# Vahe1994/AQLM

Measured on AMD Instinct MI355X. Metric: QuantizedLinear 1x16g8 matvec algorithmic GB/s (bs=1, Llama-3-8B shapes 4096->4096/11008), higher is better.
Workload: dtype f16; 1 GPU; decode step = 32 blocks x {4096->4096, 4096->11008} 1x16g8 matvec, bs=1, 64 distinct layers (own codes + codebook), 564 MB algorithmic bytes/step, hipGraph replay; scheme=1x16g8, batch=1, kernels=prepacked slice-bucketed gemv (layers of >= 0.5 M codes: both shapes), parallelism=single GPU, packed_bytes=1190264832, canonical_code_bytes=494927872

## Files before the change

aqlm_amd/_native.py:

```python
from __future__ import annotations

import ctypes
import os

_HERE = os.path.dirname(os.path.abspath(__file__))
LIB_PATH = os.environ.get("AQLM_AMD_HIP_LIB") or os.path.join(_HERE, "libaqlm_hip.so")
ABI_VERSION = 9

F16, BF16 = 0, 1
F32 = 2
E_INVALID, E_UNSUPPORTED = -1, -2
MAX_GEMV_BATCH = 8
OP_GEMM_1X16_MFMA = 1
OP_GEMV_1X16_PACKED = 3
OP_GEMV_8X8_LUT = 4
OP_GEMM_KX8_MFMA = 6
OP_GEMV_1X16_G16_PACKED = 5

MAX_SEGMENTS = 4
MAX_ROUTED_PAIRS = 64
MAX_ROUTED_EXPERTS = 256
ROUTED_ENTRY_WORDS = 4
MAX_GROUPED_PAIRS = 1 << 18
GROUPED_TILE_PAIRS = (16, 32, 64, 128)
# ... 228 lines not shown

def check(rc: int, what: str = "") -> None:
    if rc == 0:
        return
    msg = last_error() or what
    if rc == E_UNSUPPORTED:
        raise NotImplementedError(msg)
    if rc == E_INVALID:
        raise ValueError(msg)
    raise AqlmHipError(f"HIP error {rc}: {msg}")


def set_tuning(key: str, value: int) -> None:
    check(lib.aqlm_hip_set_tuning(key.encode(), int(value)), "set_tuning")


def get_tuning(key: str) -> int:
    v = _ci(0)
    check(lib.aqlm_hip_get_tuning(key.encode(), ctypes.byref(v)), "get_tuning")
    return v.value


CAPTURE_OVERLAP_FIELDS = ("seen", "relaxed", "kept_conflict", "kept_window", "runs_broken", "api_failures",
                          "merged", "merge_refused", "nodes_added")


def capture_overlap_stats(reset: bool = False) -> dict:
    out = (ctypes.c_uint64 * len(CAPTURE_OVERLAP_FIELDS))()
    check(lib.aqlm_hip_capture_overlap_stats_ex(out, len(out)), "capture_overlap_stats")
    if reset:
        check(lib.aqlm_hip_capture_overlap_stats_ex(None, 0), "capture_overlap_stats")
    return dict(zip(CAPTURE_OVERLAP_FIELDS, (int(v) for v in out)))


def packed_image(desc: "PackedDesc", rows: int = 1, dtype: int = F16):
    lds, win = _sz(0), ctypes.c_uint32(0)
    check(lib.aqlm_hip_gemv_1x16_packed_image(ctypes.byref(desc), int(rows), int(dtype), 0, ctypes.byref(lds), ctypes.byref(win), None),
          "packed_image")
    return int(lds.value), int(win.value)


def packed_image_blocks_per_cu(desc: "PackedDesc", rows: int = 1, dtype: int = F16, probe_lds_bytes: int = 0) -> int:
    n = _ci(0)
    check(lib.aqlm_hip_gemv_1x16_packed_image(ctypes.byref(desc), int(rows), int(dtype), int(probe_lds_bytes), None, None, ctypes.byref(n)),
          "packed_image")
    return n.value
```

aqlm_amd/csrc/api.hip:

```cpp
#include <stdarg.h>
#include <string.h>

#include <algorithm>
#include <map>
#include <mutex>
#include <utility>

#include "aqlm_common.h"

namespace aqlm {

static thread_local char g_err[512] = "";

void set_last_error(const char* fmt, ...) {
  va_list ap;
  va_start(ap, fmt);
  vsnprintf(g_err, sizeof(g_err), fmt, ap);
  va_end(ap);
}

int check_hip(hipError_t e, const char* what) {
  if (e == hipSuccess) return 0;
  set_last_error("%s: %s (%d)", what, hipGetErrorString(e), (int)e);
  return (int)e;
// ... 33 lines not shown
  if (!strcmp(key, "kx8_xres_phased")) return &t.kx8_xres_phased;
  if (!strcmp(key, "kx8_phase_tpb")) return &t.kx8_phase_tpb;
  if (!strcmp(key, "kx8_phase_quads")) return &t.kx8_phase_quads;
  if (!strcmp(key, "kx8_multi_xres_min_rows")) return &t.kx8_multi_xres_min_rows;
  if (!strcmp(key, "kx8_ksplit")) return &t.kx8_ksplit;
  if (!strcmp(key, "kx8_rt")) return &t.kx8_rt;
  if (!strcmp(key, "scan_max_rows")) return &t.scan_max_rows;
  if (!strcmp(key, "scan_prefetch")) return &t.scan_prefetch;
  if (!strcmp(key, "gemm_debug")) return &t.gemm_debug;
  if (!strcmp(key, "gemm_store_nt")) return &t.gemm_store_nt;
  if (!strcmp(key, "force_generic")) return &t.force_generic;
  if (!strcmp(key, "packed_waves")) return &t.packed_waves;
  if (!strcmp(key, "packed_fused_finalize")) return &t.packed_fused_finalize;
  if (!strcmp(key, "packed_prefetch")) return &t.packed_prefetch;
  if (!strcmp(key, "packed_arrange")) return &t.packed_arrange;
  if (!strcmp(key, "packed_xcopies")) return &t.packed_xcopies;
  if (!strcmp(key, "packed_entry_bytes")) return &t.packed_entry_bytes;
  if (!strcmp(key, "packed_debug")) return &t.packed_debug;
  if (!strcmp(key, "packed_fill_rotate")) return &t.packed_fill_rotate;
  if (!strcmp(key, "packed_compact_window")) return &t.packed_compact_window;
  if (!strcmp(key, "packed_capture_window")) return &t.packed_capture_window;
  if (!strcmp(key, "packed_capture_min_run")) return &t.packed_capture_min_run;
  if (!strcmp(key, "packed_capture_merge")) return &t.packed_capture_merge;
  if (!strcmp(key, "packed_pipe")) return &t.packed_pipe;
  if (!strcmp(key, "packed_prefetch_waves")) return &t.packed_prefetch_waves;
  if (!strcmp(key, "packed_dequant_by_xcd")) return &t.packed_dequant_by_xcd;
  if (!strcmp(key, "lut_waves")) return &t.lut_waves;
  return nullptr;
}

namespace {
struct CaptureOverlapState {
  std::mutex mu;
  capture_overlap::Planner planner;
  uint64_t stats[9] = {0, 0, 0, 0, 0, 0, 0, 0, 0};
  bool off = false;
};
CaptureOverlapState& capture_state() {
  static CaptureOverlapState s;
  return s;
}
hipError_t set_capture_deps(hipStream_t stream, const std::vector<capture_overlap::NodeId>& nodes) {
  static_assert(sizeof(hipGraphNode_t) == sizeof(capture_overlap::NodeId), "a graph node handle is carried as a 64-bit id");
  std::vector<hipGraphNode_t> d;
  for (capture_overlap::NodeId n : nodes) d.push_back(reinterpret_cast<hipGraphNode_t>(static_cast<uintptr_t>(n)));
  return hipStreamUpdateCaptureDependencies(stream, d.empty() ? nullptr : d.data(), d.size(), hipStreamSetCaptureDependencies);
}
bool same_nodes(const std::vector<capture_overlap::NodeId>& a, const std::vector<capture_overlap::NodeId>& b) {
  return a.size() == b.size() && std::is_permutation(a.begin(), a.end(), b.begin());
}
bool read_capture(hipStream_t stream, bool& capturing, unsigned long long& id, std::vector<capture_overlap::NodeId>& deps, hipError_t& err) {
  hipStreamCaptureStatus st = hipStreamCaptureStatusNone;
  const hipGraphNode_t* d = nullptr;
  size_t n = 0;
  hipGraph_t graph = nullptr;
  err = hipStreamGetCaptureInfo_v2(stream, &st, &id, &graph, &d, &n);
  if (err != hipSuccess) return false;
  capturing = st == hipStreamCaptureStatusActive;
// ... 46 lines not shown
  }
  fail("hipStreamUpdateCaptureDependencies", e);
  s.planner.run(id_).reset();
  active_ = false;
}

int CaptureRelax::begin(uint64_t key, const void* member, size_t member_bytes) {
  if (!active_ || begun_) return 0;
  begun_ = true;
  const int merge = std::min(std::max(tuning().packed_capture_merge, 1), capture_overlap::kMaxMerge);
  if (merge > 1 && key != 0 && member) {
    key_ = key;
    member_.assign(static_cast<const unsigned char*>(member), static_cast<const unsigned char*>(member) + member_bytes);
  }
  CaptureOverlapState& s = capture_state();
  std::lock_guard<std::mutex> lock(s.mu);
  plan_ = s.planner.run(id_).plan(before_.data(), before_.size(), fp, tuning().packed_capture_window, tuning().packed_capture_min_run,
                                  key_, merge);
  if (plan_.merge) return plan_.member;
  apply_plan();
  return 0;
}

bool CaptureRelax::join(const hipKernelNodeParams* node) {
  if (!active_ || !begun_ || done_ || !plan_.merge) return false;
  CaptureOverlapState& s = capture_state();
  std::lock_guard<std::mutex> lock(s.mu);
  capture_overlap::Run& run = s.planner.run(id_);
  const hipError_t e = node && run.latest(plan_)
                           ? hipGraphKernelNodeSetParams(reinterpret_cast<hipGraphNode_t>(static_cast<uintptr_t>(plan_.target)), node)
                           : hipErrorInvalidValue;
  if (e == hipSuccess && run.commit(plan_, plan_.target, fp, member_.data(), member_.size())) {
    ++s.stats[3];
    ++s.stats[6];
    --s.stats[8];
    done_ = true;
    return true;
  }
  (void)hipGetLastError();
  ++s.stats[7];
  plan_ = run.plan(before_.data(), before_.size(), fp, tuning().packed_capture_window, tuning().packed_capture_min_run, key_, 1);
  apply_plan();
  return false;
}

int CaptureRelax::launched() {
  if (!active_ || !begun_ || done_) return 0;
  done_ = true;
  CaptureOverlapState& s = capture_state();
  std::lock_guard<std::mutex> lock(s.mu);
  capture_overlap::Run& run = s.planner.run(id_);
  bool capturing = false;
  unsigned long long id = 0;
  std::vector<capture_overlap::NodeId> now;
  hipError_t err = hipSuccess;
  const bool read = read_capture(stream_, capturing, id, now, err);
  std::vector<capture_overlap::NodeId> want;
  if (read && capturing && id == id_ && now.size() == 1 && run.commit(plan_, now[0], std::move(fp), member_.data(), member_.size())) {
// ... 50 lines not shown
    atomicAdd(&out[1], b);
  }
}

}

extern "C" int aqlm_hip_checksum(const void* data, size_t bytes, void* out_u64x2, void* stream_) {
  hipStream_t stream = (hipStream_t)stream_;
  if (!out_u64x2 || (!data && bytes) || (reinterpret_cast<uintptr_t>(out_u64x2) & 7u)) {
    aqlm::set_last_error("aqlm_hip_checksum: null pointer argument or misaligned output");
    return AQLM_HIP_E_INVALID;
  }
  if (int e = aqlm::check_hip(hipMemsetAsync(out_u64x2, 0, 16, stream), "checksum memset")) return e;
  if (bytes == 0) return 0;
  const size_t nwords = (bytes + 3) / 4;
  const unsigned blocks = (unsigned)std::min<size_t>(2048, (nwords + 255) / 256);
  hipLaunchKernelGGL(aqlm::checksum_kernel, dim3(blocks), dim3(256), 0, stream, (const uint8_t*)data, bytes, (unsigned long long*)out_u64x2);
  return aqlm::check_hip(hipGetLastError(), "checksum launch");
}

static int capture_overlap_stats(uint64_t* out, int n) {
  aqlm::CaptureOverlapState& s = aqlm::capture_state();
  std::lock_guard<std::mutex> lock(s.mu);
  for (int i = 0; i < 9; ++i) {
    if (!out) s.stats[i] = 0;
    else if (i < n) out[i] = s.stats[i];
  }
  return 0;
}

extern "C" int aqlm_hip_capture_overlap_stats(uint64_t out[6]) { return capture_overlap_stats(out, 6); }

extern "C" int aqlm_hip_capture_overlap_stats_ex(uint64_t* out, int count) {
  if (out && (count < 0 || count > 9)) {
    aqlm::set_last_error("aqlm_hip_capture_overlap_stats_ex: count must be 0..9 (got %d)", count);
    return AQLM_HIP_E_INVALID;
  }
  return capture_overlap_stats(out, count);
}

extern "C" int aqlm_hip_abi_version(void) { return AQLM_HIP_ABI_VERSION; }

extern "C" const char* aqlm_hip_last_error(void) { return aqlm::g_err; }

extern "C" int aqlm_hip_set_tuning(const char* key, int value) {
  int* s = aqlm::tuning_slot(key);
  if (!s) {
    aqlm::set_last_error("aqlm_hip_set_tuning: unknown key '%s'", key ? key : "(null)");
    return AQLM_HIP_E_INVALID;
  }
  *s = value;
  return 0;
}

extern "C" int aqlm_hip_get_tuning(const char* key, int* value) {
  int* s = aqlm::tuning_slot(key);
  if (!s || !value) {
    aqlm::set_last_error("aqlm_hip_get_tuning: unknown key '%s'", key ? key : "(null)");
// ... 6 lines not shown
```

aqlm_amd/csrc/aqlm_common.h:

```cpp
#pragma once
#include <hip/hip_runtime.h>
#include <stdint.h>
#include <stdio.h>
#include <string.h>

#include "../../include/aqlm_hip.h"
#include "capture_overlap.h"

namespace aqlm {

constexpr int WAVE = 64;

typedef unsigned int u32x4 __attribute__((ext_vector_type(4)));
typedef unsigned int u32x2 __attribute__((ext_vector_type(2)));
typedef _Float16 f16x2 __attribute__((ext_vector_type(2)));
typedef __bf16 bf16x2 __attribute__((ext_vector_type(2)));

constexpr int AUX_DEFAULT = 0;
constexpr int AUX_SC0 = 1;
constexpr int AUX_NT = 2;
constexpr int AUX_SC1 = 16;

struct F16 {
  static constexpr int id = AQLM_HIP_F16;
  static __device__ __forceinline__ float dot2(uint32_t a, uint32_t b, float c) {
    return __builtin_amdgcn_fdot2(__builtin_bit_cast(f16x2, a), __builtin_bit_cast(f16x2, b), c, false);
  }
  static __device__ __forceinline__ float to_float(uint16_t u) { return (float)__builtin_bit_cast(_Float16, u); }
  static __device__ __forceinline__ uint16_t from_float(float f) {
    return __builtin_bit_cast(uint16_t, (_Float16)f);
// ... 105 lines not shown
  int kx8_phase_quads = 0;
  int kx8_mfma_min_rows = 2;
  int kx8_multi_xres_min_rows = 2;
  int kx8_ksplit = 0;
  int kx8_rt = 0;
  int gemm_debug = 0;
  int gemm_store_nt = 0;
  int force_generic = 0;
  int packed_fused_finalize = 1;
  int packed_waves = 0;
  int packed_arrange = 1;
  int packed_xcopies = 0;
  int packed_entry_bytes = 0;
  int packed_debug = 0;
  int packed_prefetch = 0;
  int packed_pipe = 1;
  int packed_fill_rotate = 1;
  int packed_compact_window = 0;
  int lut_waves = 0;
  int packed_prefetch_waves = 0;
  int packed_capture_window = capture_overlap::kDefaultWindow;
  int packed_capture_min_run = capture_overlap::kDefaultMinRun;
  int packed_capture_merge = capture_overlap::kDefaultMerge;
  int packed_dequant_by_xcd = 1;
};
Tuning& tuning();

class CaptureRelax {
 public:
  explicit CaptureRelax(hipStream_t stream);
  ~CaptureRelax();
  CaptureRelax(const CaptureRelax&) = delete;
  CaptureRelax& operator=(const CaptureRelax&) = delete;
  bool capturing() const { return active_; }
  capture_overlap::Footprint fp;
  int begin(uint64_t key = 0, const void* member = nullptr, size_t member_bytes = 0);
  const std::vector<unsigned char>& group() const { return plan_.payload; }
  bool join(const hipKernelNodeParams* node);
  int launched();

 private:
  void fail(const char* what, hipError_t e);
  void apply_plan();
  hipStream_t stream_;
  bool active_ = false, begun_ = false, done_ = false, changed_ = false;
  uint64_t key_ = 0;
  std::vector<unsigned char> member_;
  unsigned long long id_ = 0;
  std::vector<capture_overlap::NodeId> before_;
  capture_overlap::Plan plan_;
};

namespace scan {
size_t workspace_bytes(int B, int M, int K);
int run(const void* codes, const void* codebook, const void* scales, const void* bias, const void* X, void* Y, int batch, int out_features,
        int in_features, long xs, long ys, int dtype, void* workspace, hipStream_t stream);
}

inline bool aligned16(const void* p) { return (reinterpret_cast<uintptr_t>(p) & 15u) == 0; }
inline bool aligned8(const void* p) { return (reinterpret_cast<uintptr_t>(p) & 7u) == 0; }
inline bool ids_aligned(const void* ids, int ids_int64) { return (reinterpret_cast<uintptr_t>(ids) & (ids_int64 ? 7u : 3u)) == 0; }
// ... 49 lines not shown
```

aqlm_amd/csrc/capture_overlap.h:

```cpp
#ifndef AQLM_CAPTURE_OVERLAP_H_
#define AQLM_CAPTURE_OVERLAP_H_

#include <stddef.h>
#include <stdint.h>

#include <algorithm>
#include <vector>

namespace aqlm {
namespace capture_overlap {

using NodeId = uint64_t;

constexpr int kMaxWindow = 8;
constexpr int kDefaultWindow = 2;
constexpr int kDefaultMinRun = 8;
constexpr int kMaxMerge = 8;
constexpr int kDefaultMerge = 6;
constexpr size_t kMaxRanges = 256;

struct Range {
  uintptr_t begin, end;
  bool writes;
};

struct Footprint {
  std::vector<Range> ranges;
  void add(const void* p, size_t bytes, bool writes) {
    if (!p || !bytes) return;
    const uintptr_t b = reinterpret_cast<uintptr_t>(p);
    ranges.push_back(Range{b, b + bytes, writes});
  }
  void add_rows(const void* p, int rows, long stride_bytes, size_t row_bytes, bool writes) {
    if (rows > 1 && stride_bytes == (long)row_bytes) return add(p, (size_t)rows * row_bytes, writes);
    for (int r = 0; r < rows; ++r) add(reinterpret_cast<const char*>(p) + (ptrdiff_t)r * stride_bytes, row_bytes, writes);
  }
};

inline bool hazard(const Footprint& a, const Footprint& b) {
  for (const Range& x : a.ranges)
    for (const Range& y : b.ranges)
// ... 180 lines not shown
```

aqlm_amd/csrc/packed_gemv_entries.h:

```cpp

static bool packed_fused(const aqlm_hip_packed_desc* desc) {
  return tuning().packed_fused_finalize != 0 && desc->codebook_absmax > 0.f && desc->codebook_absmax < __builtin_inff();
}

struct PackedFused {
  const void* scales = nullptr;
  const void* bias = nullptr;
  void* y = nullptr;
  long y_row_stride = 0;
  float cb_absmax = 0.f;
  void* cells = nullptr;
  float* pub = nullptr;
  uint32_t* pub_flag = nullptr;
  uint32_t* pub_epoch = nullptr;
  uint32_t pub_max_elems = 0;
};

struct PackedNext {
  const uint8_t* ent = nullptr;
  const uint8_t* codebook = nullptr;
  uint32_t block_bytes = 0;
};

static int packed_launch_main(const PackedLayout& L, const void* packed, const void* codebook, const uint16_t* x, int nb,
// ... 24 lines not shown
  }
#ifdef AQLM_PACKED_TRACE
  rest.trace = workspace && workspace_bytes >= need + (size_t)PK_NST * PK_MAX_NW * 8 * 8 ? (unsigned long long*)((uint8_t*)workspace + need) : nullptr;
  rest.dbg = tuning().packed_debug;
#endif
  int npw = 0;
  if (next.ent && next.codebook && next.block_bytes) {
    const int want = tuning().packed_prefetch_waves < 0 ? 0 : (tuning().packed_prefetch_waves == 0 ? 2 : tuning().packed_prefetch_waves);
    npw = std::min(std::min(want, 7), PK_MAX_NW - L.NW);
  }
  const uint32_t rotate = tuning().packed_fill_rotate ? 1u : 0u;
#if AQLM_PK_G == 8
  auto try_join = [&](bool vg, const PackedGroupSegment& me, unsigned threads, size_t lds, bool& joined) -> int {
    joined = false;
    if (tuning().packed_capture_merge <= 1) {
      if (relax) relax->begin();
      return 0;
    }
    const void* gk = vg ? (dtype == AQLM_HIP_F16 ? (const void*)gemv_1x16_packed_group_kernel<F16, 3, PK_XWIN_COMPACT, 4, true>
                                                 : (const void*)gemv_1x16_packed_group_kernel<BF16, 3, PK_XWIN_COMPACT, 4, true>)
                        : (dtype == AQLM_HIP_F16 ? (const void*)gemv_1x16_packed_group_kernel<F16, 3, PK_XWIN_COMPACT, 4, false>
                                                 : (const void*)gemv_1x16_packed_group_kernel<BF16, 3, PK_XWIN_COMPACT, 4, false>);
    if (int e = ensure_dynamic_lds(gk, lds)) return e;
    if (!relax) return 0;
    uint64_t key = (uint64_t)reinterpret_cast<uintptr_t>(gk) * 0x9E3779B97F4A7C15ull ^ ((uint64_t)threads << 32) ^ (uint64_t)lds;
    if (key == 0) key = 1;
    const int n = relax->begin(key, &me, sizeof me);
    if (n <= 0) return 0;
    const std::vector<unsigned char>& members = relax->group();
    if (n >= PK_GROUP_MAX || members.size() != (size_t)n * sizeof(PackedGroupSegment)) {
      relax->join(nullptr);
      return 0;
    }
    PackedGroupParams gp{};
    memcpy(gp.seg, members.data(), members.size());
    gp.seg[n] = me;
    void* args[1] = {&gp};
    hipKernelNodeParams node{};
    node.func = const_cast<void*>(gk);
    node.gridDim = dim3((unsigned)(n + 1) * PK_NST);
    node.blockDim = dim3(threads);
    node.sharedMemBytes = (unsigned)lds;
    node.kernelParams = args;
    node.extra = nullptr;
    joined = relax->join(&node);
    return 0;
  };
#endif
  auto launch = [&](auto kern, auto lds_map) -> int {
    const size_t lds = decltype(lds_map)::total(L.in_groups, L.RG, npw, L.NW);
    if (lds > 160 * 1024) { npw = 0; }
    const size_t lds_final = decltype(lds_map)::total(L.in_groups, L.RG, npw, L.NW);
    if (int e = ensure_dynamic_lds(reinterpret_cast<const void*>(kern), lds_final)) return e;
    PackedGemvRest r = rest;
    r.pub = fused.pub;
    r.pub_flag = fused.pub_flag;
    r.pub_epoch = fused.pub_epoch;
    r.pub_max_elems = fused.pub_max_elems;
    if (npw) {
      r.next_ent = next.ent;
      r.next_codebook = next.codebook;
      r.next_block_bytes = next.block_bytes;
    }
    bool joined = false;
#if AQLM_PK_G == 8
    if (decltype(lds_map)::TIGHT && nb == 1 && npw == 0 && fused.y && !fused.pub) {
      PackedGroupSegment me{};
      me.codebook = cb;
// ... 502 lines not shown
```

aqlm_amd/csrc/packed_gemv_kernels.h:

```cpp

struct PackedGemvParams {
  const uint32_t* ent;
  const uint32_t* winfo;
  const uint32_t* rowstart;
  const uint8_t* codebook;
  const uint16_t* x;
  float* partial;
  long x_row_stride;
  int M, in_groups, RG, NW, T, XC;
  uint32_t ent_bytes;
  unsigned long long* acc;
  float cb_absmax;
  const uint16_t* scales;
  const uint16_t* bias;
  uint16_t* y;
  long y_row_stride;
  float* pub;
  uint32_t* pub_flag;
  uint32_t* pub_epoch;
  uint32_t pub_max_elems;
  const uint8_t* next_ent;
  const uint8_t* next_codebook;
  uint32_t next_block_bytes;
  int NPW;
// ... 49 lines not shown
  }
  static constexpr bool TIGHT = XFIRST && XWIN < PK_XWIN_FULL;
  __host__ __device__ static uint32_t rs_bytes(int RG) {
    return TIGHT ? ((uint32_t)(RG + 1) * 4u + 255u) & ~255u : ((uint32_t)(RG + 1) * 4u + 1023u) & ~1023u;
  }
  __host__ __device__ static uint32_t rowval(int in_groups, int RG) { return rowstart(in_groups) + rs_bytes(RG); }
  __host__ __device__ static uint32_t colend(int in_groups, int RG) { return rowval(in_groups, RG) + (uint32_t)B * (RG + 1) * 4u; }
  __host__ __device__ static uint32_t xmax(int in_groups, int RG, int nw) {
    return (colend(in_groups, RG) + (uint32_t)B * (TIGHT ? (uint32_t)nw : (uint32_t)PK_MAX_NW) * 64 * 4 + 15u) & ~15u;
  }
  __host__ __device__ static uint32_t dump(int in_groups, int RG, int nw) {
    return (xmax(in_groups, RG, nw) + (uint32_t)B * PK_MAX_NW * 4u + 15u) & ~15u;
  }
  __host__ __device__ static size_t total(int in_groups, int RG, int npw = 0, int nw = PK_MAX_NW) {
    return npw ? (size_t)dump(in_groups, RG, nw) + (size_t)npw * 1024
               : (size_t)xmax(in_groups, RG, nw) + (size_t)B * PK_MAX_NW * 4;
  }
};

struct PackedVgArgs {
  uint32_t ns[4];
};

template <class T_, int B, int PD, uint32_t XWIN, int EB, bool PUB = false, bool VG = false, bool NOPF = false>
__device__ __forceinline__ void gemv_1x16_packed_body(const PackedGemvParams& p, const int block, const int NWB,
                                                      const PackedVgArgs& vg = PackedVgArgs{}) {
  using LDS = PackedLds<B, XWIN>;
  using ring_t = typename std::conditional<EB == 3, u32x3, u32x4>::type;
  extern __shared__ __attribute__((aligned(16))) unsigned char smem_raw[];
  const int tid = threadIdx.x, lane = tid & 63;
  const int NT = NWB << 6;
  const int wave = __builtin_amdgcn_readfirstlane(tid >> 6);
#ifdef AQLM_PACKED_TRACE
  unsigned long long tr[8];
  uint32_t tr_wait = 0, tr_work = 0;
  tr[0] = wall_clock64();
  const unsigned long long cyc0 = __builtin_readcyclecounter();
#define AQLM_TRACE(i) tr[i] = wall_clock64()
#else
#define AQLM_TRACE(i)
#endif
  int slice, group, row_begin, nrows, stream_ix;
  if constexpr (VG) {
    static_assert(PK_S == 16 && PK_NST == 256, "variable geometry: 16 slices, 256 workgroups");
    stream_ix = ((block & 7) << 5) | (block >> 3);
    const uint32_t w = lane < 4 ? vg.ns[0] : (lane < 8 ? vg.ns[1] : (lane < 12 ? vg.ns[2] : vg.ns[3]));
    const uint32_t start_v = (w >> ((lane & 3) * 8)) & 255u;
    const unsigned long long m = __ballot((uint32_t)stream_ix >= start_v) & 0xffffull;
    const int s = __popcll(m) - 1;
// ... 6 lines not shown
    const int base = p.M / n, extra = p.M - base * n;
    row_begin = group * base + (group < extra ? group : extra);
    nrows = base + (group < extra ? 1 : 0);
  } else {
    stream_ix = block;
    slice = block & (PK_S - 1);
    group = block >> PK_S_LOG;
    row_begin = group * p.RG;
    nrows = p.M - row_begin;
    nrows = nrows < 0 ? 0 : (nrows < p.RG ? nrows : p.RG);
  }
  if ((uint32_t)(size_t)(__attribute__((address_space(3))) unsigned char*)smem_raw != 0u) __builtin_trap();

  const int RG1 = p.RG + 1;
  const uint32_t rowstart_off = LDS::rowstart(p.in_groups);
  const uint32_t rowval_off = LDS::rowval(p.in_groups, p.RG);
  const uint32_t colend_off = LDS::colend(p.in_groups, p.RG);

  const uint32_t XP = LDS::plane(p.in_groups);
  const uint32_t xstride16 = (uint32_t)pk_x_stride(p.in_groups) * PK_VB;
  __amdgpu_buffer_rsrc_t rs_ent = __builtin_amdgcn_make_buffer_rsrc((void*)p.ent, 0, p.ent_bytes, 0x00020000);
  const int wv = wave < p.NW ? wave : p.NW - 1;
  const uint32_t wbase = (uint32_t)(((size_t)stream_ix * p.NW + wv) * p.T) * (EB == 3 ? (uint32_t)PK_WREG3 : 1024u);
  const int Tm1 = p.T - 1;
  u32x2 flagw = {0u, 0u};
  if constexpr (EB == 3)
    flagw = __builtin_amdgcn_raw_buffer_load_b64(rs_ent, (uint32_t)(lane < Tm1 ? lane : Tm1) * 8u, wbase, 0);
  const int NWD = NWB - p.NPW;
  const bool pfw = !NOPF && wave >= NWD;
  if (pfw) {
    const int pw = wave - NWD;
    const uint32_t dump = LDS::dump(p.in_groups, p.RG, p.NW) + (uint32_t)pw * 1024u;
    const uint8_t* nsrc = p.next_ent + (size_t)block * p.next_block_bytes;
    for (uint32_t off = (uint32_t)pw * 1024u; off < p.next_block_bytes; off += (uint32_t)p.NPW * 1024u)
      __builtin_amdgcn_global_load_lds((gbl_void_ptr)(nsrc + off + lane * 16), (lds_void_ptr)(size_t)dump, 16, 0, AUX_NT);
    constexpr uint32_t SHARE = PK_SLICE_BYTES / PK_NG;
    const uint8_t* csrc = p.next_codebook + (size_t)slice * PK_SLICE_BYTES + (size_t)group * SHARE;
    for (uint32_t off = (uint32_t)pw * 1024u; off < SHARE; off += (uint32_t)p.NPW * 1024u)
      __builtin_amdgcn_global_load_lds((gbl_void_ptr)(csrc + off + lane * 16), (lds_void_ptr)(size_t)dump, 16, 0, 0);
  }
  if (!pfw) {
    const uint8_t* src = p.codebook + (size_t)slice * PK_SLICE_BYTES;
    constexpr int PIECES = (int)(PK_SLICE_BYTES / 1024);
    const int rot = p.fill_rotate ? (group & (PK_NG - 1)) * (PIECES / PK_NG) : 0;
    for (int i0 = wave; i0 < PIECES; i0 += NWD) {
      const int i = (i0 + rot) & (PIECES - 1);
      __builtin_amdgcn_global_load_lds((gbl_void_ptr)(src + i * 1024 + lane * 16),
                                       (lds_void_ptr)(size_t)(LDS::SLICE + (uint32_t)i * 1024u), 16, 0, 0);
    }
    const int x16 = p.in_groups * (int)(PK_VB / 16);
    const int nchunk = (x16 + 63) >> 6;
    const int ncopy = B == 1 ? p.XC : B;
    for (int c = wave; c < nchunk * ncopy; c += NWD) {
      const int b = c / nchunk, i = c - b * nchunk;
      const int idx = i * 64 + lane;
      const uint32_t dst = LDS::X + (uint32_t)b * (B == 1 ? xstride16 : XP) + (uint32_t)i * 1024u;
      if (idx < x16)
        __builtin_amdgcn_global_load_lds((gbl_void_ptr)(p.x + (B == 1 ? (size_t)0 : (size_t)b * p.x_row_stride) + (size_t)idx * 8),
                                         (lds_void_ptr)(size_t)dst, 16, 0, 0);
    }
    const uint32_t* rs_src = p.rowstart + (size_t)stream_ix * RG1;
    for (int i = wave; i * 64 < RG1; i += NWD) {
      const int idx = i * 64 + lane;
      if (idx < RG1)
        __builtin_amdgcn_global_load_lds((gbl_void_ptr)(rs_src + idx), (lds_void_ptr)(size_t)(rowstart_off + (uint32_t)i * 256u), 4, 0, 0);
    }
  }
  const uint32_t voff = (uint32_t)lane * (EB == 3 ? 12u : 16u);
  const uint32_t ebase = EB == 3 ? wbase + (uint32_t)p.T * 8u : wbase;
  auto fetch = [&](int t) -> ring_t {
#ifdef AQLM_PACKED_TRACE
    const uint32_t vo = (t <= Tm1 && !(p.dbg & 2)) ? voff : 0xfffffff0u;
#else
    const uint32_t vo = t <= Tm1 ? voff : 0xfffffff0u;
#endif
    if constexpr (EB == 3) return __builtin_amdgcn_raw_buffer_load_b96(rs_ent, vo, ebase + (uint32_t)t * (uint32_t)PK_STEP3, AUX_NT);
    else return __builtin_amdgcn_raw_buffer_load_b128(rs_ent, vo, ebase + (uint32_t)t * 1024u, AUX_NT);
  };
  ring_t ring[PD];
#pragma unroll
  for (int k = 0; k < PD; ++k) ring[k] = fetch(pfw ? 0x7fffffff : k);
  int steps = wave < p.NW ? p.T : 0;
  [[maybe_unused]] uint32_t wave_start_row = 0u;
  if constexpr (EB == 3) {
    const const_u32_ptr wi = (const_u32_ptr)(uintptr_t)(p.winfo + ((size_t)stream_ix * p.NW + wv) * 4);
    steps = wave < p.NW ? (int)wi[2] : 0;
    wave_start_row = wi[3];
  }
  if (tid < B * (int)(PK_VB / 16))
    *reinterpret_cast<u32x4*>(smem_raw + LDS::X + (uint32_t)(tid / (int)(PK_VB / 16)) * XP + (uint32_t)p.in_groups * PK_VB +
                              (uint32_t)(tid % (int)(PK_VB / 16)) * 16u) = u32x4{0u, 0u, 0u, 0u};
  const uint32_t xmax_off = LDS::xmax(p.in_groups, p.RG, p.NW);
  if (tid < B * PK_MAX_NW) *reinterpret_cast<uint32_t*>(smem_raw + xmax_off + (uint32_t)tid * 4u) = 0u;
  AQLM_TRACE(1);
  asm volatile("" : : "s"(p.acc), "s"(p.partial), "s"(p.scales), "s"(p.bias), "s"(p.y), "s"(p.y_row_stride), "s"(p.cb_absmax));
  uint16_t scale_h, bias_h;
  {
    const int r = tid < nrows ? tid : (nrows > 0 ? nrows - 1 : 0);
    const uint16_t* sp = p.scales ? p.scales : reinterpret_cast<const uint16_t*>(p.rowstart);
    const uint16_t* bp = p.bias ? p.bias : sp;
    scale_h = sp[row_begin + r];
    bias_h = bp[row_begin + r];
  }
  constexpr int PDW = PD + 2;
  if (!pfw) __builtin_amdgcn_s_waitcnt((PDW & 15) | (7 << 4) | (0 << 8) | ((PDW >> 4) << 14));
  else __builtin_amdgcn_s_waitcnt(63 | (7 << 4) | (0 << 8) | (3 << 14));
  __builtin_amdgcn_s_barrier();
  AQLM_TRACE(2);

  uint32_t mask = PK_HMASK;
  asm volatile("" : "+v"(mask));
  constexpr int NA = 1;
  float acc[B][NA];
#pragma unroll
  for (int b = 0; b < B; ++b)
#pragma unroll
    for (int a = 0; a < NA; ++a) acc[b][a] = 0.f;
  uint32_t row_addr = 0;

  constexpr int NV = (int)(PK_VB / 16);
  constexpr int EG0 = B <= 2 ? 4 : (B <= 4 ? 2 : 1);
  constexpr int EG = NV > 1 && EG0 > 1 && B > 1 ? EG0 / 2 : EG0;
  auto entries = [&](const uint32_t (&a_cb)[4], const uint32_t (&a_x)[4], const uint32_t (&copy)[4]) {
#ifdef AQLM_PACKED_TRACE
    if (p.dbg & 1) { acc[0][0] += __uint_as_float(a_cb[0] ^ a_x[1] ^ a_cb[2] ^ a_x[3]); return; }
#endif
#pragma unroll
// ... 70 lines not shown
        a_x[k] = half_and<1>(w[k], mask);
        if constexpr (B > 1) copy[k] = (w[k] >> 16) & 3u;
      }
      entries(a_cb, a_x, copy);
      if (e.x & 1u) flush();
    } else {
      const uint32_t w0 = e.x, w1 = e.y, w2 = e.z;
      const uint32_t t1 = __builtin_amdgcn_alignbit(w1, w0, 24);
      const uint32_t t2 = __builtin_amdgcn_alignbit(w2, w1, 28);
      a_cb[0] = (w0 << 4) & 0xfff0u;   a_x[0] = (w0 >> 8) & 0xfff0u;
      a_cb[1] = (t1 << 4) & 0xfff0u;   a_x[1] = w1 & 0xfff0u;
      a_cb[2] = (w1 >> 12) & 0xfff0u;  a_x[2] = (t2 << 4) & 0xfff0u;
      a_cb[3] = (w2 >> 4) & 0xfff0u;   a_x[3] = half_and<1>(w2, mask);
      if constexpr (B > 1) {
#pragma unroll
        for (int k = 0; k < 4; ++k) copy[k] = __umulhi(a_x[k] >> 4, xrecip);
      }
      entries(a_cb, a_x, copy);
      if (cmask & 1u) flush();
      cmask >>= 1;
    }
  };

  if (steps > 0) {
    if constexpr (EB == 4) {
      const uint32_t f = pk_get_start_row(ring[0].x, ring[0].y, ring[0].z, ring[0].w);
      row_addr = rowval_off + f * 4u;
    } else {
      uint32_t pre = 0u;
      const uint32_t l31 = (uint32_t)lane & 31u;
      for (int t = 0; t < steps; ++t) {
        const uint32_t slo = (uint32_t)__builtin_amdgcn_readlane((int)flagw.x, t), shi = (uint32_t)__builtin_amdgcn_readlane((int)flagw.y, t);
        const uint32_t sel = lane >= 32 ? shi : slo;
        cmask |= ((sel >> l31) & 1u) << t;
        pre = __builtin_amdgcn_mbcnt_hi(shi, __builtin_amdgcn_mbcnt_lo(slo, pre));
      }
      row_addr = rowval_off + (wave_start_row + pre) * 4u;
    }
    int t = 0;
    for (; t + PD <= steps; t += PD) {
#pragma unroll
      for (int k = 0; k < PD; ++k) {
#ifdef AQLM_PACKED_TRACE
        const unsigned long long c0 = __builtin_amdgcn_s_memtime();
        __builtin_amdgcn_s_waitcnt(((PD - 1) & 15) | (7 << 4) | (15 << 8));
        const unsigned long long c1 = __builtin_amdgcn_s_memtime();
        step(ring[k]);
        asm volatile("s_waitcnt lgkmcnt(0)" ::: "memory");
        const unsigned long long c2 = __builtin_amdgcn_s_memtime();
        tr_wait += (uint32_t)(c1 - c0);
        tr_work += (uint32_t)(c2 - c1);
#else
        step(ring[k]);
#endif
        ring[k] = fetch(t + PD + k);
      }
    }
    const int rem = steps - t;
#pragma unroll
    for (int k = 0; k < PD - 1; ++k)
      if (k < rem) step(ring[k]);
  }
  if (p.acc != nullptr) {
    typedef unsigned short us2 __attribute__((ext_vector_type(2)));
#pragma unroll
    for (int b = 0; b < B; ++b) {
      us2 m = {0, 0};
      for (int idx = tid; idx < p.in_groups * (int)(PK_VB / 16); idx += NT) {
        const u32x4 v = *(lds_u32x4_ptr)(size_t)(LDS::X + (uint32_t)b * (B == 1 ? 0u : XP) + (uint32_t)idx * 16u);
        const uint32_t w[4] = {v.x, v.y, v.z, v.w};
#pragma unroll
        for (int k = 0; k < 4; ++k) m = __builtin_elementwise_max(m, __builtin_bit_cast(us2, w[k] & 0x7fff7fffu));
      }
      const uint32_t mm = wave_max_u32(m.x > m.y ? (uint32_t)m.x : (uint32_t)m.y);
      if (lane == 0) *reinterpret_cast<uint32_t*>(smem_raw + xmax_off + (uint32_t)(b * PK_MAX_NW + wave) * 4u) = mm;
    }
  }

  if (wave < p.NW) {
#pragma unroll
    for (int b = 0; b < B; ++b) lds_store_f32(colend_off + (uint32_t)((b * PK_MAX_NW + wave) * 64 + lane) * 4u, total(b));
  }
  AQLM_TRACE(4);
  asm volatile("s_waitcnt lgkmcnt(0)" : : : "memory");
  __syncthreads();
  AQLM_TRACE(5);
  float* pub_half = nullptr;
  uint32_t pub_e = 0u;
  if (PUB && p.pub != nullptr && p.acc != nullptr) {
    pub_e = __hip_atomic_load(p.pub_epoch, __ATOMIC_RELAXED, __HIP_MEMORY_SCOPE_AGENT);
    pub_half = p.pub + (size_t)(pub_e & 1u) * p.pub_max_elems;
  }
  {
    const uint32_t* rs = reinterpret_cast<const uint32_t*>(smem_raw + rowstart_off);
    const float* rowval = reinterpret_cast<const float*>(smem_raw + rowval_off);
    const float* colend = reinterpret_cast<const float*>(smem_raw + colend_off);
    const uint32_t T = (uint32_t)p.T;
    for (int r = tid; r < nrows; r += NT) {
      const uint32_t q0 = rs[r], q1 = rs[r + 1];
      const uint32_t c0 = q0 / T, c1 = (q1 - 1u) / T;
      float v[B];
#pragma unroll
      for (int b = 0; b < B; ++b) {
        v[b] = rowval[b * RG1 + r];
        for (uint32_t c = c0; c < c1; ++c) v[b] += colend[(size_t)b * PK_MAX_NW * 64 + c];
      }
      if (p.acc == nullptr) {
#pragma unroll
        for (int b = 0; b < B; ++b) p.partial[((size_t)slice * B + b) * p.M + row_begin + r] = v[b];
      } else {
        const int row = row_begin + r;
        unsigned long long old[B], mine[B];
        int sh[B];
#pragma unroll
        for (int b = 0; b < B; ++b) {
          uint32_t xm = 0u;
          {
            static_assert(PK_MAX_NW == 16, "four 16-byte reads cover the slots");
            u32x4 sl[4];
#pragma unroll
            for (int q = 0; q < 4; ++q) sl[q] = *(lds_u32x4_ptr)(size_t)(xmax_off + (uint32_t)(b * PK_MAX_NW + q * 4) * 4u);
#pragma unroll
            for (int q = 0; q < 4; ++q) {
              const uint32_t a = sl[q].x > sl[q].y ? sl[q].x : sl[q].y, c = sl[q].z > sl[q].w ? sl[q].z : sl[q].w;
              const uint32_t d = a > c ? a : c;
              xm = d > xm ? d : xm;
            }
          }
          const float bound = (float)p.in_groups * (float)PK_G * p.cb_absmax * T_::to_float((uint16_t)xm);
          int e = 0;
          (void)frexpf(bound, &e);
          const bool finite = bound < __builtin_inff() && fabsf(v[b]) <= 2.f * bound;
          sh[b] = PK_FIX_BITS - e;
          const long long q = finite ? __float2ll_rn(ldexpf(v[b], sh[b])) : 0ll;
          mine[b] = ((unsigned long long)q << PK_VAL_SHIFT) + (finite ? 1ull : 1ull + (1ull << PK_CNT_BITS));
          old[b] = __hip_atomic_fetch_add(p.acc + (size_t)b * p.M + row, mine[b], __ATOMIC_RELAXED, __HIP_MEMORY_SCOPE_AGENT);
        }
        const bool first = r == tid;
        const float scale = pub_half ? 1.f : T_::to_float(first ? scale_h : p.scales[row]);
        const float bias = (pub_half || !p.bias) ? 0.f : T_::to_float(first ? bias_h : p.bias[row]);
#pragma unroll
        for (int b = 0; b < B; ++b) {
          if ((old[b] & PK_CNT_MASK) == (unsigned long long)(PK_S - 1)) {
            const unsigned long long cell = old[b] + mine[b];
            const long long sum = (long long)cell >> PK_VAL_SHIFT;
            float sv = (float)ldexp((double)sum, -sh[b]);
            if ((cell >> PK_CNT_BITS) & PK_CNT_MASK) sv = __builtin_nanf("");
            if (pub_half)
              __hip_atomic_store(pub_half + (size_t)b * p.M + row, sv, __ATOMIC_RELAXED, __HIP_MEMORY_SCOPE_SYSTEM);
            else
              p.y[(size_t)b * p.y_row_stride + row] = T_::from_float(__builtin_fmaf(sv, scale, bias));
            __hip_atomic_store(p.acc + (size_t)b * p.M + row, 0ull, __ATOMIC_RELAXED, __HIP_MEMORY_SCOPE_AGENT);
          }
        }
      }
    }
  }
  if (pub_half) {
    asm volatile("s_waitcnt vmcnt(0)" ::: "memory");
    __syncthreads();
    if (tid == 0) {
      uint32_t* shard = p.pub_epoch + 4 + (block & 7);
      const uint32_t a = __hip_atomic_fetch_add(shard, 1u, __ATOMIC_RELAXED, __HIP_MEMORY_SCOPE_AGENT);
      if (a + 1u == (uint32_t)(PK_NST / 8)) {
        __hip_atomic_store(shard, 0u, __ATOMIC_RELAXED, __HIP_MEMORY_SCOPE_AGENT);
        const uint32_t t = __hip_atomic_fetch_add(p.pub_epoch + 12, 1u, __ATOMIC_RELAXED, __HIP_MEMORY_SCOPE_AGENT);
        if (t + 1u == 8u) {
          __hip_atomic_store(p.pub_epoch + 12, 0u, __ATOMIC_RELAXED, __HIP_MEMORY_SCOPE_AGENT);
          __builtin_amdgcn_fence(__ATOMIC_RELEASE, "");
          asm volatile("s_waitcnt vmcnt(0)" ::: "memory");
          __hip_atomic_store(p.pub_flag + (pub_e & 1u), pub_e, __ATOMIC_RELAXED, __HIP_MEMORY_SCOPE_SYSTEM);
        }
      }
    }
  }
#ifdef AQLM_PACKED_TRACE
  AQLM_TRACE(6);
  if (p.trace && lane == 0) {
    unsigned long long* o = p.trace + ((size_t)block * PK_MAX_NW + wave) * 8;
    tr[3] = __builtin_readcyclecounter() - cyc0;
    tr[7] = ((unsigned long long)tr_wait << 32) | tr_work;
    for (int i = 0; i < 8; ++i) o[i] = tr[i];
  }
#endif
}

struct PackedGemvRest {
  const uint32_t* winfo;
  float* partial;
  long x_row_stride;
  unsigned long long* acc;
  const uint16_t* scales;
  const uint16_t* bias;
  uint16_t* y;
  long y_row_stride;
  float cb_absmax;
// ... 192 lines not shown
    vg.ns[1] = s->ns[1];
    vg.ns[2] = s->ns[2];
    vg.ns[3] = s->ns[3];
  }
  p.winfo = s->rest.winfo;
  p.partial = s->rest.partial;
  p.x_row_stride = s->rest.x_row_stride;
  p.acc = s->rest.acc;
  p.cb_absmax = s->rest.cb_absmax;
  p.scales = s->rest.scales;
  p.bias = s->rest.bias;
  p.y = s->rest.y;
  p.y_row_stride = s->rest.y_row_stride;
#ifdef AQLM_PACKED_TRACE
  p.trace = s->rest.trace;
  p.dbg = s->rest.dbg;
#endif
  p.NW = (int)(geom & 0xffu);
  p.XC = (int)((geom >> 8) & 0xfu);
  p.fill_rotate = (int)((geom >> 15) & 1u);
  p.T = (int)(geom >> 16);
  gemv_1x16_packed_body<T_, 1, PD, XWIN, EB, false, VG>(p, (int)blockIdx.x % PK_NST, (int)blockDim.x >> 6, vg);
}
#endif

struct PackedFinalizeParams {
  const float* partial;
  const uint16_t* scales;
  const uint16_t* bias;
  uint16_t* y;
  long y_row_stride;
  int M, B;
};

template <class T_>
__device__ __forceinline__ void packed_finalize_row(const PackedFinalizeParams& p, int row) {
  if (row >= p.M) return;
  const float scale = T_::to_float(p.scales[row]);
  const float bias = p.bias ? T_::to_float(p.bias[row]) : 0.f;
  for (int b = 0; b < p.B; ++b) {
    float s = 0.f;
#pragma unroll
    for (int k = 0; k < PK_S; ++k) s += p.partial[((size_t)k * p.B + b) * p.M + row];
    p.y[(size_t)b * p.y_row_stride + row] = T_::from_float(__builtin_fmaf(s, scale, bias));
  }
}
// ... 39 lines not shown
```

Before: 1689 GB/s.

## Fold multiple row groups per block in merged packed gemv group launches

New measurement: 1918 GB/s (median of 6 runs). 13.6% higher.

```diff
diff --git a/aqlm_amd/_native.py b/aqlm_amd/_native.py
--- a/aqlm_amd/_native.py
+++ b/aqlm_amd/_native.py
@@ -274,7 +274,7 @@
 
 
 CAPTURE_OVERLAP_FIELDS = ("seen", "relaxed", "kept_conflict", "kept_window", "runs_broken", "api_failures",
-                          "merged", "merge_refused", "nodes_added")
+                          "merged", "merge_refused", "nodes_added", "folded")
 
 
 def capture_overlap_stats(reset: bool = False) -> dict:
diff --git a/aqlm_amd/csrc/api.hip b/aqlm_amd/csrc/api.hip
--- a/aqlm_amd/csrc/api.hip
+++ b/aqlm_amd/csrc/api.hip
@@ -79,6 +79,7 @@
   if (!strcmp(key, "packed_capture_window")) return &t.packed_capture_window;
   if (!strcmp(key, "packed_capture_min_run")) return &t.packed_capture_min_run;
   if (!strcmp(key, "packed_capture_merge")) return &t.packed_capture_merge;
+  if (!strcmp(key, "packed_group_fold")) return &t.packed_group_fold;
   if (!strcmp(key, "packed_pipe")) return &t.packed_pipe;
   if (!strcmp(key, "packed_prefetch_waves")) return &t.packed_prefetch_waves;
   if (!strcmp(key, "packed_dequant_by_xcd")) return &t.packed_dequant_by_xcd;
@@ -90,7 +91,7 @@
 struct CaptureOverlapState {
   std::mutex mu;
   capture_overlap::Planner planner;
-  uint64_t stats[9] = {0, 0, 0, 0, 0, 0, 0, 0, 0};
+  uint64_t stats[10] = {0, 0, 0, 0, 0, 0, 0, 0, 0, 0};
   bool off = false;
 };
 CaptureOverlapState& capture_state() {
@@ -183,7 +184,7 @@
   return 0;
 }
 
-bool CaptureRelax::join(const hipKernelNodeParams* node) {
+bool CaptureRelax::join(const hipKernelNodeParams* node, int folded_delta) {
   if (!active_ || !begun_ || done_ || !plan_.merge) return false;
   CaptureOverlapState& s = capture_state();
   std::lock_guard<std::mutex> lock(s.mu);
@@ -195,6 +196,7 @@
     ++s.stats[3];
     ++s.stats[6];
     --s.stats[8];
+    s.stats[9] += (uint64_t)(int64_t)folded_delta;
     done_ = true;
     return true;
   }
@@ -291,7 +293,7 @@
 static int capture_overlap_stats(uint64_t* out, int n) {
   aqlm::CaptureOverlapState& s = aqlm::capture_state();
   std::lock_guard<std::mutex> lock(s.mu);
-  for (int i = 0; i < 9; ++i) {
+  for (int i = 0; i < 10; ++i) {
     if (!out) s.stats[i] = 0;
     else if (i < n) out[i] = s.stats[i];
   }
@@ -301,8 +303,8 @@
 extern "C" int aqlm_hip_capture_overlap_stats(uint64_t out[6]) { return capture_overlap_stats(out, 6); }
 
 extern "C" int aqlm_hip_capture_overlap_stats_ex(uint64_t* out, int count) {
-  if (out && (count < 0 || count > 9)) {
-    aqlm::set_last_error("aqlm_hip_capture_overlap_stats_ex: count must be 0..9 (got %d)", count);
+  if (out && (count < 0 || count > 10)) {
+    aqlm::set_last_error("aqlm_hip_capture_overlap_stats_ex: count must be 0..10 (got %d)", count);
     return AQLM_HIP_E_INVALID;
   }
   return capture_overlap_stats(out, count);
diff --git a/aqlm_amd/csrc/aqlm_common.h b/aqlm_amd/csrc/aqlm_common.h
--- a/aqlm_amd/csrc/aqlm_common.h
+++ b/aqlm_amd/csrc/aqlm_common.h
@@ -6,6 +6,7 @@
 
 #include "../../include/aqlm_hip.h"
 #include "capture_overlap.h"
+#include "group_fold.h"
 
 namespace aqlm {
 
@@ -157,6 +158,7 @@
   int packed_capture_window = capture_overlap::kDefaultWindow;
   int packed_capture_min_run = capture_overlap::kDefaultMinRun;
   int packed_capture_merge = capture_overlap::kDefaultMerge;
+  int packed_group_fold = 0;
   int packed_dequant_by_xcd = 1;
 };
 Tuning& tuning();
@@ -171,7 +173,7 @@
   capture_overlap::Footprint fp;
   int begin(uint64_t key = 0, const void* member = nullptr, size_t member_bytes = 0);
   const std::vector<unsigned char>& group() const { return plan_.payload; }
-  bool join(const hipKernelNodeParams* node);
+  bool join(const hipKernelNodeParams* node, int folded_delta = 0);
   int launched();
 
  private:
diff --git a/aqlm_amd/csrc/capture_overlap.h b/aqlm_amd/csrc/capture_overlap.h
--- a/aqlm_amd/csrc/capture_overlap.h
+++ b/aqlm_amd/csrc/capture_overlap.h
@@ -16,7 +16,7 @@
 constexpr int kDefaultWindow = 2;
 constexpr int kDefaultMinRun = 8;
 constexpr int kMaxMerge = 8;
-constexpr int kDefaultMerge = 6;
+constexpr int kDefaultMerge = 4;
 constexpr size_t kMaxRanges = 256;
 
 struct Range {
diff --git a/aqlm_amd/csrc/group_fold.h b/aqlm_amd/csrc/group_fold.h
--- /dev/null
+++ b/aqlm_amd/csrc/group_fold.h
@@ -0,0 +1,45 @@
+#ifndef AQLM_GROUP_FOLD_H_
+#define AQLM_GROUP_FOLD_H_
+
+#if defined(__HIPCC__) || defined(__CUDACC__)
+#define AQLM_FOLD_HD __host__ __device__
+#else
+#define AQLM_FOLD_HD
+#endif
+
+namespace aqlm {
+namespace group_fold {
+
+constexpr int kSlices = 16, kGroups = 16, kStreams = kSlices * kGroups;
+constexpr int kDefaultFold = 4;
+
+struct Place {
+  int segment;
+  int slice;
+  int first_group;
+  int group_step;
+};
+
+AQLM_FOLD_HD inline bool valid(int fold) { return fold == 1 || fold == 2 || fold == 4; }
+AQLM_FOLD_HD inline unsigned grid(int members, int fold) { return (unsigned)members * (unsigned)(kStreams / fold); }
+
+AQLM_FOLD_HD inline Place place(unsigned block, int fold) {
+  const unsigned shift = 8u - ((unsigned)fold >> 1);
+  const unsigned b = block & ((1u << shift) - 1u);
+  Place q;
+  q.segment = (int)(block >> shift);
+  q.slice = (int)(b & (unsigned)(kSlices - 1));
+  q.first_group = (int)(b >> 4);
+  q.group_step = kGroups >> ((unsigned)fold >> 1);
+  return q;
+}
+AQLM_FOLD_HD inline int stream(const Place& q, int pass) { return (q.first_group + pass * q.group_step) * kSlices + q.slice; }
+
+AQLM_FOLD_HD inline int choose(int key, int members) {
+  const int f = key == 0 ? kDefaultFold : key;
+  return valid(f) && members >= f ? f : 1;
+}
+
+}
+}
+#endif
diff --git a/aqlm_amd/csrc/packed_gemv_entries.h b/aqlm_amd/csrc/packed_gemv_entries.h
--- a/aqlm_amd/csrc/packed_gemv_entries.h
+++ b/aqlm_amd/csrc/packed_gemv_entries.h
@@ -70,6 +70,11 @@
                         : (dtype == AQLM_HIP_F16 ? (const void*)gemv_1x16_packed_group_kernel<F16, 3, PK_XWIN_COMPACT, 4, false>
                                                  : (const void*)gemv_1x16_packed_group_kernel<BF16, 3, PK_XWIN_COMPACT, 4, false>);
     if (int e = ensure_dynamic_lds(gk, lds)) return e;
+    const void* fk = vg ? nullptr
+                        : (dtype == AQLM_HIP_F16 ? (const void*)gemv_1x16_packed_group_fold_kernel<F16, 3, PK_XWIN_COMPACT, 4>
+                                                 : (const void*)gemv_1x16_packed_group_fold_kernel<BF16, 3, PK_XWIN_COMPACT, 4>);
+    if (fk)
+      if (int e = ensure_dynamic_lds(fk, lds)) return e;
     if (!relax) return 0;
     uint64_t key = (uint64_t)reinterpret_cast<uintptr_t>(gk) * 0x9E3779B97F4A7C15ull ^ ((uint64_t)threads << 32) ^ (uint64_t)lds;
     if (key == 0) key = 1;
@@ -83,15 +88,20 @@
     PackedGroupParams gp{};
     memcpy(gp.seg, members.data(), members.size());
     gp.seg[n] = me;
-    void* args[1] = {&gp};
+    const int key_fold = tuning().packed_group_fold;
+    bool one_row_before = fk != nullptr;
+    for (int i = 0; i < n; ++i) one_row_before = one_row_before && gp.seg[i].RG <= (int)threads;
+    const bool was_folded = one_row_before && group_fold::choose(key_fold, n) > 1;
+    int fold = one_row_before && me.RG <= (int)threads ? group_fold::choose(key_fold, n + 1) : 1;
+    void* args[2] = {&gp, &fold};
     hipKernelNodeParams node{};
-    node.func = const_cast<void*>(gk);
-    node.gridDim = dim3((unsigned)(n + 1) * PK_NST);
+    node.func = const_cast<void*>(fold > 1 ? fk : gk);
+    node.gridDim = dim3(group_fold::grid(n + 1, fold));
     node.blockDim = dim3(threads);
     node.sharedMemBytes = (unsigned)lds;
     node.kernelParams = args;
     node.extra = nullptr;
-    joined = relax->join(&node);
+    joined = relax->join(&node, (fold > 1 ? 1 : 0) - (was_folded ? 1 : 0));
     return 0;
   };
 #endif
diff --git a/aqlm_amd/csrc/packed_gemv_kernels.h b/aqlm_amd/csrc/packed_gemv_kernels.h
--- a/aqlm_amd/csrc/packed_gemv_kernels.h
+++ b/aqlm_amd/csrc/packed_gemv_kernels.h
@@ -95,9 +95,11 @@
   uint32_t ns[4];
 };
 
-template <class T_, int B, int PD, uint32_t XWIN, int EB, bool PUB = false, bool VG = false, bool NOPF = false>
+template <class T_, int B, int PD, uint32_t XWIN, int EB, bool PUB = false, bool VG = false, bool NOPF = false, bool FOLD = false>
 __device__ __forceinline__ void gemv_1x16_packed_body(const PackedGemvParams& p, const int block, const int NWB,
-                                                      const PackedVgArgs& vg = PackedVgArgs{}) {
+                                                      const PackedVgArgs& vg = PackedVgArgs{}, const int npass = 1,
+                                                      const int group_step = 0) {
+  static_assert(!FOLD || (B == 1 && EB == 4 && !PUB && !VG && NOPF), "folded launch: one row, 4-byte entries, ordinary geometry");
   using LDS = PackedLds<B, XWIN>;
   using ring_t = typename std::conditional<EB == 3, u32x3, u32x4>::type;
   extern __shared__ __attribute__((aligned(16))) unsigned char smem_raw[];
@@ -150,7 +152,7 @@
   __amdgpu_buffer_rsrc_t rs_ent = __builtin_amdgcn_make_buffer_rsrc((void*)p.ent, 0, p.ent_bytes, 0x00020000);
   const int wv = wave < p.NW ? wave : p.NW - 1;
   const uint32_t wbase = (uint32_t)(((size_t)stream_ix * p.NW + wv) * p.T) * (EB == 3 ? (uint32_t)PK_WREG3 : 1024u);
-  const int Tm1 = p.T - 1;
+  int Tm1 = p.T - 1;
   u32x2 flagw = {0u, 0u};
   if constexpr (EB == 3)
     flagw = __builtin_amdgcn_raw_buffer_load_b64(rs_ent, (uint32_t)(lane < Tm1 ? lane : Tm1) * 8u, wbase, 0);
@@ -187,15 +189,17 @@
         __builtin_amdgcn_global_load_lds((gbl_void_ptr)(p.x + (B == 1 ? (size_t)0 : (size_t)b * p.x_row_stride) + (size_t)idx * 8),
                                          (lds_void_ptr)(size_t)dst, 16, 0, 0);
     }
-    const uint32_t* rs_src = p.rowstart + (size_t)stream_ix * RG1;
-    for (int i = wave; i * 64 < RG1; i += NWD) {
-      const int idx = i * 64 + lane;
-      if (idx < RG1)
-        __builtin_amdgcn_global_load_lds((gbl_void_ptr)(rs_src + idx), (lds_void_ptr)(size_t)(rowstart_off + (uint32_t)i * 256u), 4, 0, 0);
+    if constexpr (!FOLD) {
+      const uint32_t* rs_src = p.rowstart + (size_t)stream_ix * RG1;
+      for (int i = wave; i * 64 < RG1; i += NWD) {
+        const int idx = i * 64 + lane;
+        if (idx < RG1)
+          __builtin_amdgcn_global_load_lds((gbl_void_ptr)(rs_src + idx), (lds_void_ptr)(size_t)(rowstart_off + (uint32_t)i * 256u), 4, 0, 0);
+      }
     }
   }
   const uint32_t voff = (uint32_t)lane * (EB == 3 ? 12u : 16u);
-  const uint32_t ebase = EB == 3 ? wbase + (uint32_t)p.T * 8u : wbase;
+  uint32_t ebase = EB == 3 ? wbase + (uint32_t)p.T * 8u : wbase;
   auto fetch = [&](int t) -> ring_t {
 #ifdef AQLM_PACKED_TRACE
     const uint32_t vo = (t <= Tm1 && !(p.dbg & 2)) ? voff : 0xfffffff0u;
@@ -223,14 +227,32 @@
   AQLM_TRACE(1);
   asm volatile("" : : "s"(p.acc), "s"(p.partial), "s"(p.scales), "s"(p.bias), "s"(p.y), "s"(p.y_row_stride), "s"(p.cb_absmax));
   uint16_t scale_h, bias_h;
-  {
+  [[maybe_unused]] uint32_t q0_h = 0u, q1_h = 0u;
+  [[maybe_unused]] auto pass_loads = [&](int g, uint16_t& sc, uint16_t& bi, uint32_t& q0, uint32_t& q1) {
+    const int rb = g * p.RG;
+    int n = p.M - rb;
+    n = n < 0 ? 0 : (n < p.RG ? n : p.RG);
+    const int r = tid < n ? tid : (n > 0 ? n - 1 : 0);
+    const int row = rb + r < p.M ? rb + r : p.M - 1;
+    const uint16_t* bp = p.bias ? p.bias : p.scales;
+    const uint32_t* rs_g = p.rowstart + (size_t)(g * PK_S + slice) * RG1;
+    sc = p.scales[row];
+    bi = bp[row];
+    typedef uint32_t rs_pair __attribute__((ext_vector_type(2), aligned(4)));
+    const rs_pair q = *reinterpret_cast<const rs_pair*>(rs_g + r);
+    q0 = q.x;
+    q1 = q.y;
+  };
+  if constexpr (FOLD) {
+    pass_loads(group, scale_h, bias_h, q0_h, q1_h);
+  } else {
     const int r = tid < nrows ? tid : (nrows > 0 ? nrows - 1 : 0);
     const uint16_t* sp = p.scales ? p.scales : reinterpret_cast<const uint16_t*>(p.rowstart);
     const uint16_t* bp = p.bias ? p.bias : sp;
     scale_h = sp[row_begin + r];
     bias_h = bp[row_begin + r];
   }
-  constexpr int PDW = PD + 2;
+  constexpr int PDW = PD + (FOLD ? 3 : 2);
   if (!pfw) __builtin_amdgcn_s_waitcnt((PDW & 15) | (7 << 4) | (0 << 8) | ((PDW >> 4) << 14));
   else __builtin_amdgcn_s_waitcnt(63 | (7 << 4) | (0 << 8) | (3 << 14));
   __builtin_amdgcn_s_barrier();
@@ -347,6 +369,8 @@
     }
   };
 
+  [[maybe_unused]] int pass = 0;
+next_pass:
   if (steps > 0) {
     if constexpr (EB == 4) {
       const uint32_t f = pk_get_start_row(ring[0].x, ring[0].y, ring[0].z, ring[0].w);
@@ -386,7 +410,7 @@
     for (int k = 0; k < PD - 1; ++k)
       if (k < rem) step(ring[k]);
   }
-  if (p.acc != nullptr) {
+  if (p.acc != nullptr && (!FOLD || pass == 0)) {
     typedef unsigned short us2 __attribute__((ext_vector_type(2)));
 #pragma unroll
     for (int b = 0; b < B; ++b) {
@@ -410,6 +434,17 @@
   asm volatile("s_waitcnt lgkmcnt(0)" : : : "memory");
   __syncthreads();
   AQLM_TRACE(5);
+  [[maybe_unused]] uint16_t scale_n = 0, bias_n = 0;
+  [[maybe_unused]] uint32_t q0_n = 0u, q1_n = 0u;
+  if constexpr (FOLD) {
+    const bool more = pass + 1 < npass;
+    const int g = more ? group + group_step : group;
+    pass_loads(g, scale_n, bias_n, q0_n, q1_n);
+    ebase = (uint32_t)(((size_t)(g * PK_S + slice) * p.NW + wv) * p.T) * 1024u;
+    Tm1 = more ? p.T - 1 : -1;
+#pragma unroll
+    for (int k = 0; k < PD; ++k) ring[k] = fetch(k);
+  }
   float* pub_half = nullptr;
   uint32_t pub_e = 0u;
   if (PUB && p.pub != nullptr && p.acc != nullptr) {
@@ -422,7 +457,14 @@
     const float* colend = reinterpret_cast<const float*>(smem_raw + colend_off);
     const uint32_t T = (uint32_t)p.T;
     for (int r = tid; r < nrows; r += NT) {
-      const uint32_t q0 = rs[r], q1 = rs[r + 1];
+      uint32_t q0, q1;
+      if constexpr (FOLD) {
+        q0 = q0_h;
+        q1 = q1_h;
+      } else {
+        q0 = rs[r];
+        q1 = rs[r + 1];
+      }
       const uint32_t c0 = q0 / T, c1 = (q1 - 1u) / T;
       float v[B];
 #pragma unroll
@@ -461,7 +503,7 @@
           mine[b] = ((unsigned long long)q << PK_VAL_SHIFT) + (finite ? 1ull : 1ull + (1ull << PK_CNT_BITS));
           old[b] = __hip_atomic_fetch_add(p.acc + (size_t)b * p.M + row, mine[b], __ATOMIC_RELAXED, __HIP_MEMORY_SCOPE_AGENT);
         }
-        const bool first = r == tid;
+        const bool first = FOLD || r == tid;
         const float scale = pub_half ? 1.f : T_::to_float(first ? scale_h : p.scales[row]);
         const float bias = (pub_half || !p.bias) ? 0.f : T_::to_float(first ? bias_h : p.bias[row]);
 #pragma unroll
@@ -497,6 +539,27 @@
           __hip_atomic_store(p.pub_flag + (pub_e & 1u), pub_e, __ATOMIC_RELAXED, __HIP_MEMORY_SCOPE_SYSTEM);
         }
       }
+    }
+  }
+  if constexpr (FOLD) {
+    if (++pass < npass) {
+      group += group_step;
+      stream_ix = group * PK_S + slice;
+      row_begin = group * p.RG;
+      nrows = p.M - row_begin;
+      nrows = nrows < 0 ? 0 : (nrows < p.RG ? nrows : p.RG);
+      scale_h = scale_n;
+      bias_h = bias_n;
+      q0_h = q0_n;
+      q1_h = q1_n;
+#pragma unroll
+      for (int b = 0; b < B; ++b)
+#pragma unroll
+        for (int a = 0; a < NA; ++a) acc[b][a] = 0.f;
+      row_addr = 0;
+      asm volatile("s_waitcnt lgkmcnt(0)" : : : "memory");
+      __builtin_amdgcn_s_barrier();
+      goto next_pass;
     }
   }
 #ifdef AQLM_PACKED_TRACE
@@ -735,6 +798,43 @@
   p.T = (int)(geom >> 16);
   gemv_1x16_packed_body<T_, 1, PD, XWIN, EB, false, VG>(p, (int)blockIdx.x % PK_NST, (int)blockDim.x >> 6, vg);
 }
+
+template <class T_, int PD, uint32_t XWIN, int EB>
+__global__ __launch_bounds__(1024) void gemv_1x16_packed_group_fold_kernel(const PackedGroupParams gp, const int fold) {
+  (void)gp;
+  static_assert(PK_S == group_fold::kSlices && PK_NST == group_fold::kStreams, "group_fold.h: 16 slices x 16 row groups");
+  const group_fold::Place at = group_fold::place(blockIdx.x, fold);
+  const group_segment_ptr s = (group_segment_ptr)__builtin_amdgcn_kernarg_segment_ptr() + at.segment;
+  PackedGemvParams p{};
+  p.codebook = s->codebook;
+  p.x = s->x;
+  p.ent = s->ent;
+  p.rowstart = s->rowstart;
+  p.in_groups = s->in_groups;
+  p.RG = s->RG;
+  p.M = s->M;
+  const uint32_t geom = s->geom;
+  p.ent_bytes = s->ent_bytes;
+  p.winfo = s->rest.winfo;
+  p.partial = s->rest.partial;
+  p.x_row_stride = s->rest.x_row_stride;
+  p.acc = s->rest.acc;
+  p.cb_absmax = s->rest.cb_absmax;
+  p.scales = s->rest.scales;
+  p.bias = s->rest.bias;
+  p.y = s->rest.y;
+  p.y_row_stride = s->rest.y_row_stride;
+#ifdef AQLM_PACKED_TRACE
+  p.trace = s->rest.trace;
+  p.dbg = s->rest.dbg;
+#endif
+  p.NW = (int)(geom & 0xffu);
+  p.XC = (int)((geom >> 8) & 0xfu);
+  p.fill_rotate = (int)((geom >> 15) & 1u);
+  p.T = (int)(geom >> 16);
+  gemv_1x16_packed_body<T_, 1, PD, XWIN, EB, false, false, true, true>(p, group_fold::stream(at, 0), (int)blockDim.x >> 6, PackedVgArgs{},
+                                                                       fold, at.group_step);
+}
 #endif
 
 struct PackedFinalizeParams {
```
